# mehta-lab/VisCy

Measured on AMD Instinct MI355X. Metric: training patches/sec (Z=5, 256x256, 1->2ch UNeXt2), higher is better.
Workload: dtype bf16; 1 GPU; UNeXt2 2.5D convnextv2_tiny Z=5 256x256 1->2ch, fwd+MixedLoss(0.5,0,0.5)+bwd+AdamW; per_gpu_batch=512, global_batch=512, parallelism=dp1

## Files before the change

### include/vsx.h

```cpp
#ifndef VSX_H
#define VSX_H
#include <stddef.h>
#include <stdint.h>

#ifdef __cplusplus
extern "C" {
#endif

typedef void* vsx_stream_t;

#define VSX_F32 0
#define VSX_BF16 1

int32_t vsx_version(void);
const char* vsx_last_error(void);
const char* vsx_last_kernel(void);
int32_t vsx_set_flag(const char* name, int32_t value);
int32_t vsx_get_flag(const char* name);
int32_t vsx_det_workspace(float* ws, int64_t floats);
int32_t vsx_det_scope(int32_t on);
int32_t vsx_det_active(void);

#define VSX_A_ROWS 0
#define VSX_A_PATCH2 1
// ... 206 lines not shown
#define VSX_LOSS_SLOT_STRIDE 32
int32_t vsx_loss_tmax(const float* T, int64_t n, float* tmax, vsx_stream_t stream);
int32_t vsx_ssim_scale_fwd_fused(const float* P, const float* T, const float* tmax, float* sum_ssim, float* sum_cs, float* dmu,
                                 float* Po, float* To, float* tmax_next, float* l1sum, float* l2sum, int32_t B, int32_t C,
                                 int32_t D, int32_t H, int32_t W, int32_t last, vsx_stream_t stream);
int32_t vsx_loss_finalize(const float* sum_ssim, const float* sum_cs, const float* l1sum, const float* l2sum,
    const float* npix, float nelem, int32_t B, int32_t nscale, int32_t sum_slots, float a1, float a2, float a3,
    const float* gout, float* loss, float* coef, float* ms_out, vsx_stream_t stream);

int32_t vsx_ln_fwd(const void* x, void* y, float* mean, float* rstd, const float* gamma, const float* beta,
    int32_t rows, int32_t C, float eps, int32_t dtype, vsx_stream_t stream);

int32_t vsx_ln_bwd(const void* dy, const void* x, const float* mean, const float* rstd, const float* gamma,
    const void* add, void* dx, float* dgamma, float* dbeta, int32_t rows, int32_t C, int32_t dtype,
    vsx_stream_t stream);

int32_t vsx_grn_scale(const float* colsq, const float* gamma, float* s, int32_t nb, int32_t N, float eps,
    vsx_stream_t stream);

int32_t vsx_grn_bwd_stats(const float* colsq, const float* P, const float* Sb, const float* gamma, float* t,
    float* dgamma, float* dbeta, float* rowst, int32_t nb, int32_t N, float eps, vsx_stream_t stream);

int32_t vsx_grn_gelu_bwd(void* dz, const void* h, const float* s, const float* t, float* colsum, float* ws,
    int32_t ws_rows, int32_t M, int32_t N, int32_t hw, int32_t dtype, vsx_stream_t stream);

int32_t vsx_adamw(float* p, const float* g, float* m, float* v, const float* hyper, int64_t n,
    vsx_stream_t stream);

int32_t vsx_mlp_supported(int32_t C, int32_t hw, int64_t M, int32_t dtype);
int64_t vsx_mlp_det_floats(int32_t C, int32_t hw, int64_t M, int32_t mode);
// ... 197 lines not shown
```

### viscy_amd/_lib.py

```python

from __future__ import annotations

import ctypes as C
import os

import torch

_HERE = os.path.dirname(os.path.abspath(__file__))
LIB_PATH = os.environ.get("VSX_LIB", os.path.join(_HERE, "libvsx.so"))

VSX_F32, VSX_BF16 = 0, 1
A_ROWS, A_PATCH2, A_CONV3 = 0, 1, 2
PRO_NONE, PRO_GRN = 0, 1
EPI_NONE, EPI_BIAS, EPI_BIAS_GELU_SQ, EPI_BIAS_RES, EPI_DZ, EPI_BIAS_STATS, EPI_LN_BWD = 0, 1, 2, 3, 4, 5, 6
LOSS_SLOTS, LOSS_SLOT_STRIDE = 64, 32
SPOTLIGHT_CHUNK = 16384
SPOTLIGHT_THRESHOLD, SPOTLIGHT_MASK_U8, SPOTLIGHT_MASK_F32 = 0, 1, 2
SPOTLIGHT_WS_FWD, SPOTLIGHT_WS_OTSU = 0, 1

_I32, _F32, _P, _I64 = C.c_int32, C.c_float, C.c_void_p, C.c_int64


class VsxGemm(C.Structure):
    _fields_ = [
# ... 35 lines not shown
    "vsx_version": (_I32, []),
    "vsx_weight_tasks": (_I32, [_P, _I32, _P]),
    "vsx_last_error": (C.c_char_p, []),
    "vsx_last_kernel": (C.c_char_p, []),
    "vsx_set_flag": (_I32, [C.c_char_p, _I32]),
    "vsx_get_flag": (_I32, [C.c_char_p]),
    "vsx_det_workspace": (_I32, [_P, _I64]),
    "vsx_det_scope": (_I32, [_I32]),
    "vsx_det_active": (_I32, []),
    "vsx_gemm_nt": (_I32, [C.POINTER(VsxGemm), _I32, _P]),
    "vsx_gemm_tn": (_I32, [C.POINTER(VsxGemm), _I32, _P]),
    "vsx_gemm_plan": (_I32, [_I32, C.POINTER(VsxGemm), _I32, C.POINTER(VsxGemmPlan)]),
    "vsx_gemm_nt_ln_bwd_supported": (_I32, [_I64, _I32, _I32, _I32]),
    "vsx_ln_fwd": (_I32, [_P, _P, _P, _P, _P, _P, _I32, _I32, _F32, _I32, _P]),
    "vsx_ln_bwd": (_I32, [_P, _P, _P, _P, _P, _P, _P, _P, _P, _I32, _I32, _I32, _P]),
    "vsx_grn_scale": (_I32, [_P, _P, _P, _I32, _I32, _F32, _P]),
    "vsx_grn_bwd_stats": (_I32, [_P, _P, _P, _P, _P, _P, _P, _P, _I32, _I32, _F32, _P]),
    "vsx_grn_gelu_bwd": (_I32, [_P, _P, _P, _P, _P, _P, _I32, _I32, _I32, _I32, _I32, _P]),
    "vsx_dwconv7_fwd": (_I32, [_P, _P, _P, _P, _P, _I32, _I32, _I32, _I32, _I32, _P]),
    "vsx_dwconv7_bwd_data": (_I32, [_P, _P, _P, _P, _I32, _I32, _I32, _I32, _I32, _P]),
    "vsx_dwconv7_bwd_weight": (_I32, [_P, _P, _P, _P, _P, _I32, _I32, _I32, _I32, _I32, _I32, _P]),
    "vsx_stem_im2col": (_I32, [_P, _P, _P, _P, _I32, _I32, _I32, _I32, _I32, _I32, _I32, _I32, _I32, _P]),
    "vsx_stem_im2col_ld": (_I32, [_P, _P, _P, _P, _I32, _I32, _I32, _I32, _I32, _I32, _I32, _I32, _I32, _I32, _P]),
    "vsx_pad_cols": (_I32, [_P, _P, _I32, _I32, _I32, _I32, _P]),
    "vsx_im2col3x3": (_I32, [_P, _P, _I32, _I32, _I32, _I32, _I32, _P]),
    "vsx_col2im3x3": (_I32, [_P, _P, _I32, _I32, _I32, _I32, _I32, _P]),
    "vsx_pixel_shuffle_cat_fwd": (_I32, [_P, _P, _P, _I32, _I32, _I32, _I32, _I32, _I32, _P]),
    "vsx_pixel_shuffle_cat_bwd": (_I32, [_P, _P, _P, _I32, _I32, _I32, _I32, _I32, _I32, _P]),
    "vsx_head_shuffle_fwd": (_I32, [_P, _P, _I32, _I32, _I32, _I32, _I32, _I32, _I32, _P]),
    "vsx_head_shuffle_bwd": (_I32, [_P, _P, _I32, _I32, _I32, _I32, _I32, _I32, _I32, _P]),
# ... 179 lines not shown
```

### viscy_amd/csrc/dwconv.hip

```cpp
#include "vsx_common.h"
#include "../../include/vsx.h"

template <typename T, int NCV, int TH, int TW, int K, bool FLIP>
__global__ __launch_bounds__(256) void dwconv7_kernel(const T* __restrict__ x, const float* __restrict__ w,
                                                      const float* __restrict__ bias, const T* __restrict__ add,
                                                      T* __restrict__ y, int B, int H, int W, int C) {
  constexpr int VN = VT<T>::N;
  constexpr int CB = NCV * VN;
  constexpr int PITCH = CB * (int)sizeof(T) + 16;
  constexpr int IH = TH + 6, IW = TW + 6;
  constexpr int SPR = TW / K;
  static_assert(NCV * TH * SPR == 256, "thread mapping");
  typedef typename VT<T>::vec vec;
  __shared__ __attribute__((aligned(16))) char tile[IH * IW * PITCH];
  __shared__ __attribute__((aligned(16))) float wl[49 * CB];

  const int ncb = (C + CB - 1) / CB;
  const int tiles_x = (W + TW - 1) / TW, tiles_y = (H + TH - 1) / TH;
  int bid = blockIdx.x;
  if ((gridDim.x & 7) == 0) bid = (bid & 7) * (gridDim.x >> 3) + (bid >> 3);
  const int cb = bid % ncb; bid /= ncb;
  const int tx = bid % tiles_x; bid /= tiles_x;
  const int ty = bid % tiles_y;
  const int b = bid / tiles_y;
// ... 59 lines not shown
      const int gx = x0 + sx * K + o;
      if (gx < W) {
        const size_t off = (((size_t)b * H + gy) * W + gx) * C + c0;
        if (add) {
          float a[VN];
          unpack<T>(ldvec<T>(add + off), a);
#pragma unroll
          for (int j = 0; j < VN; ++j) acc[o][j] += a[j];
        }
        stvec<T>(y + off, pack<T>(acc[o]));
      }
    }
  }
}


template <typename T, int NCV, int TH, int TW>
__global__ __launch_bounds__(256) void dwconv7_wgrad_kernel(const T* __restrict__ dy, const T* __restrict__ x,
                                                            float* __restrict__ ws, int B, int H, int W, int C,
                                                            int ngroups) {
  constexpr int VN = VT<T>::N;
  constexpr int CB = NCV * VN;
  constexpr int PITCH = CB * (int)sizeof(T) + 16;
  constexpr int IH = TH + 6, IW = TW + 6;
  constexpr int XT_BYTES = IH * IW * PITCH, DT_BYTES = TH * TW * PITCH;
  static_assert(NCV * 7 * TH <= 256, "thread mapping");
  typedef typename VT<T>::vec vec;
  constexpr int CR = 2;
  constexpr int PART_BYTES = CR * 50 * CB * 4;
  constexpr int SMEM_BYTES = XT_BYTES + DT_BYTES > PART_BYTES ? XT_BYTES + DT_BYTES : PART_BYTES;
  __shared__ __attribute__((aligned(16))) char smem[SMEM_BYTES];
  char* xt = smem;
// ... 7 lines not shown
  const int tiles_x = (W + TW - 1) / TW, tiles_y = (H + TH - 1) / TH;
  const int ntiles = B * tiles_y * tiles_x;

  const int cv = threadIdx.x % NCV;
  const int ky = (threadIdx.x / NCV) % 7;
  const int row = threadIdx.x / (NCV * 7);
  const bool worker = row < TH;
  float acc[7][VN], bsum[VN];
#pragma unroll
  for (int k = 0; k < 7; ++k)
#pragma unroll
    for (int j = 0; j < VN; ++j) acc[k][j] = 0.f;
#pragma unroll
  for (int j = 0; j < VN; ++j) bsum[j] = 0.f;

  for (int tile = group; tile < ntiles; tile += ngroups) {
    int t = tile;
    const int tx = t % tiles_x; t /= tiles_x;
    const int ty = t % tiles_y;
    const int b = t / tiles_y;
    const int y0 = ty * TH, x0 = tx * TW;
    __syncthreads();
    for (int i = threadIdx.x; i < IH * IW * NCV; i += 256) {
      const int c = i % NCV, p = i / NCV;
      const int ix = p % IW, iy = p / IW;
      const int gy = y0 + iy - 3, gx = x0 + ix - 3;
      vec v = vzero<T>();
      if (gy >= 0 && gy < H && gx >= 0 && gx < W && c_base + c * VN < C)
        v = ldvec<T>(x + (((size_t)b * H + gy) * W + gx) * C + c_base + c * VN);
      *reinterpret_cast<vec*>(xt + p * PITCH + c * 16) = v;
    }
    for (int i = threadIdx.x; i < TH * TW * NCV; i += 256) {
      const int c = i % NCV, p = i / NCV;
      const int ix = p % TW, iy = p / TW;
      const int gy = y0 + iy, gx = x0 + ix;
      vec v = vzero<T>();
      if (gy < H && gx < W && c_base + c * VN < C)
        v = ldvec<T>(dy + (((size_t)b * H + gy) * W + gx) * C + c_base + c * VN);
      *reinterpret_cast<vec*>(dt + p * PITCH + c * 16) = v;
    }
    __syncthreads();
    if (worker) {
      const char* xr = xt + ((row + ky) * IW) * PITCH + cv * 16;
      const char* dr = dt + (row * TW) * PITCH + cv * 16;
      float win[7][VN];
#pragma unroll
      for (int i = 0; i < 6; ++i) unpack<T>(*reinterpret_cast<const vec*>(xr + i * PITCH), win[i]);
#pragma unroll 1
      for (int ob = 0; ob < TW; ob += 7) {
#pragma unroll
        for (int u = 0; u < 7; ++u) {
          const int o = ob + u;
          if (o < TW) {
            unpack<T>(*reinterpret_cast<const vec*>(xr + (o + 6) * PITCH), win[(u + 6) % 7]);
            float d[VN];
            unpack<T>(*reinterpret_cast<const vec*>(dr + o * PITCH), d);
            if (ky == 3) {
#pragma unroll
              for (int j = 0; j < VN; ++j) bsum[j] += d[j];
            }
#pragma unroll
            for (int kx = 0; kx < 7; ++kx)
#pragma unroll
              for (int j = 0; j < VN; ++j) acc[kx][j] = fmaf(d[j], win[(u + kx) % 7][j], acc[kx][j]);
          }
        }
      }
    }
  }
  float* part = reinterpret_cast<float*>(smem);
  constexpr int NV = (50 * CB + 255) / 256;
  float tot[NV];
#pragma unroll
  for (int q = 0; q < NV; ++q) tot[q] = 0.f;
  for (int r0 = 0; r0 < TH; r0 += CR) {
    __syncthreads();
    if (worker && row >= r0 && row < r0 + CR) {
      float* pr = part + (size_t)(row - r0) * 50 * CB;
#pragma unroll
      for (int kx = 0; kx < 7; ++kx)
#pragma unroll
        for (int j = 0; j < VN; j += 4)
          *reinterpret_cast<float4*>(pr + (ky * 7 + kx) * CB + cv * VN + j) =
// ... 51 lines not shown
}

template <typename T, int NCV, int TH, int TW, int K>
static int dw_launch_cfg(const void* x, const float* w, const float* bias, const void* add, void* y, int B, int H, int W,
                         int C, bool flip, hipStream_t s) {
  constexpr int CB = NCV * VT<T>::N;
  long blocks = (long)B * vsx_cdiv(H, TH) * vsx_cdiv(W, TW) * vsx_cdiv(C, CB);
  dim3 grid((unsigned)blocks);
  if (flip)
    hipLaunchKernelGGL((dwconv7_kernel<T, NCV, TH, TW, K, true>), grid, dim3(256), 0, s, (const T*)x, w, bias,
                       (const T*)add, (T*)y, B, H, W, C);
  else
    hipLaunchKernelGGL((dwconv7_kernel<T, NCV, TH, TW, K, false>), grid, dim3(256), 0, s, (const T*)x, w, bias,
                       (const T*)add, (T*)y, B, H, W, C);
  VSX_LAUNCH_CHECK();
  return 0;
}

template <typename T>
static int dw_launch(const void* x, const float* w, const float* bias, const void* add, void* y, int B, int H, int W,
                     int C, bool flip, hipStream_t s);
int vsx_dwconv7_mfma_try(const void* x, const float* w, const float* bias, const void* add, void* y, int B, int H, int W, int C,
                         bool flip, hipStream_t s, int* taken);
int vsx_dwconv7_wgrad_mfma_try(const void* dy, const void* x, float* ws, int ws_rows, int B, int H, int W, int C,
                               hipStream_t s, int* taken);
template <>
int dw_launch<bf16_t>(const void* x, const float* w, const float* bias, const void* add, void* y, int B, int H, int W,
                      int C, bool flip, hipStream_t s) {
  int taken = 0;
  if (int rc = vsx_dwconv7_mfma_try(x, w, bias, add, y, B, H, W, C, flip, s, &taken)) return rc;
  if (taken) return 0;
  if (W >= 24) return dw_launch_cfg<bf16_t, 4, 8, 32, 4>(x, w, bias, add, y, B, H, W, C, flip, s);
  return dw_launch_cfg<bf16_t, 8, 8, 8, 2>(x, w, bias, add, y, B, H, W, C, flip, s);
}
template <>
int dw_launch<float>(const void* x, const float* w, const float* bias, const void* add, void* y, int B, int H, int W,
                     int C, bool flip, hipStream_t s) {
  if (W >= 24) return dw_launch_cfg<float, 8, 4, 32, 4>(x, w, bias, add, y, B, H, W, C, flip, s);
  return dw_launch_cfg<float, 8, 8, 8, 2>(x, w, bias, add, y, B, H, W, C, flip, s);
}

extern "C" int32_t vsx_dwconv7_fwd(const void* x, const float* w, const float* bias, const void* add, void* y, int32_t B,
                                   int32_t H, int32_t W, int32_t C, int32_t dtype, vsx_stream_t stream) {
  int vn = dtype == VSX_BF16 ? 8 : 4;
  VSX_CHECK(x && w && y && B > 0 && H > 0 && W > 0 && C > 0 && C % vn == 0, "vsx_dwconv7_fwd: bad arguments (C=%d)", C);
  return dtype == VSX_BF16 ? dw_launch<bf16_t>(x, w, bias, add, y, B, H, W, C, false, (hipStream_t)stream)
                           : dw_launch<float>(x, w, bias, add, y, B, H, W, C, false, (hipStream_t)stream);
}
extern "C" int32_t vsx_dwconv7_bwd_data(const void* dy, const float* w, const void* add, void* dx, int32_t B, int32_t H,
                                        int32_t W, int32_t C, int32_t dtype, vsx_stream_t stream) {
  int vn = dtype == VSX_BF16 ? 8 : 4;
  VSX_CHECK(dy && w && dx && B > 0 && H > 0 && W > 0 && C > 0 && C % vn == 0, "vsx_dwconv7_bwd_data: bad arguments");
  return dtype == VSX_BF16 ? dw_launch<bf16_t>(dy, w, nullptr, add, dx, B, H, W, C, true, (hipStream_t)stream)
                           : dw_launch<float>(dy, w, nullptr, add, dx, B, H, W, C, true, (hipStream_t)stream);
}
template <typename T, int NCV, int TH, int TW>
static int dw_wgrad_cfg(const void* dy, const void* x, float* dw, float* db, float* ws, int ws_rows, int B, int H, int W,
                        int C, hipStream_t st) {
  constexpr int CB = NCV * VT<T>::N;
  const int ncb = vsx_cdiv(C, CB);
  const int ntiles = B * vsx_cdiv(H, TH) * vsx_cdiv(W, TW);
  int ngroups = ntiles < ws_rows ? ntiles : ws_rows;
  if ((long)ngroups * ncb > 4096) ngroups = (int)(4096 / ncb) > 0 ? (int)(4096 / ncb) : 1;
  hipLaunchKernelGGL((dwconv7_wgrad_kernel<T, NCV, TH, TW>), dim3(ngroups * ncb), dim3(256), 0, st, (const T*)dy,
                     (const T*)x, ws, B, H, W, C, ngroups);
  VSX_LAUNCH_CHECK();
  hipLaunchKernelGGL(dw_reduce_rows_kernel, dim3(vsx_cdiv(50 * C, 64), vsx_cdiv(ngroups, 64)), dim3(256), 0, st, ws, dw, db,
                     ngroups, C);
  VSX_LAUNCH_CHECK();
  return 0;
}

extern "C" int32_t vsx_dwconv7_bwd_weight(const void* dy, const void* x, float* dw, float* db, float* ws, int32_t ws_rows,
                                          int32_t B, int32_t H, int32_t W, int32_t C, int32_t dtype,
                                          vsx_stream_t stream) {
  int vn = dtype == VSX_BF16 ? 8 : 4;
  VSX_CHECK(dy && x && dw && ws && ws_rows > 0 && B > 0 && H > 0 && W > 0 && C > 0 && C % vn == 0,
            "vsx_dwconv7_bwd_weight: bad arguments");
  hipStream_t st = (hipStream_t)stream;
  if (dtype == VSX_BF16) {
    int rows = 0;
    if (int rc = vsx_dwconv7_wgrad_mfma_try(dy, x, ws, ws_rows, B, H, W, C, st, &rows)) return rc;
    if (rows > 0) {
      hipLaunchKernelGGL(dw_reduce_rows_kernel, dim3(vsx_cdiv(50 * C, 64), vsx_cdiv(rows, 64)), dim3(256), 0, st, ws, dw, db, rows,
                         C);
      VSX_LAUNCH_CHECK();
      return 0;
    }
    if (W >= 24) return dw_wgrad_cfg<bf16_t, 4, 8, 16>(dy, x, dw, db, ws, ws_rows, B, H, W, C, st);
    return dw_wgrad_cfg<bf16_t, 4, 8, 8>(dy, x, dw, db, ws, ws_rows, B, H, W, C, st);
  }
  if (W >= 24) return dw_wgrad_cfg<float, 4, 8, 32>(dy, x, dw, db, ws, ws_rows, B, H, W, C, st);
  return dw_wgrad_cfg<float, 4, 8, 8>(dy, x, dw, db, ws, ws_rows, B, H, W, C, st);
}
```

### viscy_amd/csrc/norm.hip

```cpp
#include "vsx_common.h"
#include "wtasks.h"
#include "../../include/vsx.h"

template <typename T, int G, int CPL>
__global__ __launch_bounds__(256) void ln_fwd_kernel(const T* __restrict__ x, T* __restrict__ y,
                                                     float* __restrict__ mean_out, float* __restrict__ rstd_out,
                                                     const float* __restrict__ gamma, const float* __restrict__ beta,
                                                     int rows, int C, float eps, int iters, int nt) {
  constexpr int VN = VT<T>::N;
  constexpr int R = CPL == 1 ? 4 : (CPL == 2 ? 2 : 1);
  constexpr int RPI = 256 / G;
  const int nch = C / VN;
  const int gl = threadIdx.x % G;
  float gam[CPL][VN], bet[CPL][VN];
#pragma unroll
  for (int i = 0; i < CPL; ++i) {
    const int c = gl + i * G;
#pragma unroll
    for (int j = 0; j < VN; ++j) {
      gam[i][j] = (gamma && c < nch) ? gamma[c * VN + j] : 1.f;
      bet[i][j] = (gamma && c < nch) ? beta[c * VN + j] : 0.f;
    }
  }
  for (int it = 0; it < iters; ++it) {
// ... 53 lines not shown
      if (gl == 0) {
        if (mean_out) mean_out[row] = mean;
        rstd_out[row] = rstd;
      }
#endif
    }
  }
  }
}

template <typename T, int G, int CPL, bool AFF>
__global__ __launch_bounds__(256) void ln_bwd_kernel(const T* __restrict__ dy, const T* __restrict__ x,
                                                     const float* __restrict__ mean, const float* __restrict__ rstd,
                                                     const float* __restrict__ gamma, const T* __restrict__ add,
                                                     T* __restrict__ dx, float* __restrict__ dgamma,
                                                     float* __restrict__ dbeta, int rows, int C, int iters, int nt) {
  constexpr int VN = VT<T>::N;
  const bool g_nt = nt != 0;
  extern __shared__ float red[];
  const int nch = C / VN;
  const int gl = threadIdx.x % G;
  const int rslot = threadIdx.x / G;
  constexpr int RPI = 256 / G;
  if (AFF && dgamma) {
    for (int i = threadIdx.x; i < 2 * C; i += 256) red[i] = 0.f;
    __syncthreads();
  }
  constexpr int CA = AFF ? CPL : 1, VA = AFF ? VN : 1;
  float dg[CA][VA], db[CA][VA], gam[CA][VA];
  if constexpr (AFF) {
#pragma unroll
    for (int i = 0; i < CPL; ++i) {
      int c = gl + i * G;
#pragma unroll
      for (int j = 0; j < VN; ++j) {
        dg[i][j] = 0.f;
        db[i][j] = 0.f;
        gam[i][j] = (gamma && c < nch) ? gamma[c * VN + j] : 1.f;
      }
    }
  }
  typedef typename VT<T>::vec vec;
// ... 59 lines not shown
            float o[VN];
#pragma unroll
            for (int j = 0; j < VN; ++j) o[j] = rs * (g[i][j] - s1 - xh[i][j] * s2);
            if (add) {
              float a[VN];
              unpack<T>(ar[r][i], a);
#pragma unroll
              for (int j = 0; j < VN; ++j) o[j] += a[j];
            }
            stvec<T>(dx + (size_t)row * C + c * VN, pack<T>(o));
          }
        }
      }
    }
  }
  if constexpr (AFF) if (dgamma) {
#pragma unroll
    for (int i = 0; i < CPL; ++i) {
      int c = gl + i * G;
      if (c < nch) {
#pragma unroll
        for (int j = 0; j < VN; ++j) {
          atomicAdd(&red[c * VN + j], dg[i][j]);
          atomicAdd(&red[C + c * VN + j], db[i][j]);
        }
      }
    }
    __syncthreads();
    for (int i = threadIdx.x; i < C; i += 256) {
      atomicAdd(dgamma + i, red[i]);
      atomicAdd(dbeta + i, red[C + i]);
    }
  }
}

template <typename T, int G, int CPL>
static int ln_launch(bool fwd, const void* a0, const void* a1, void* out, float* mean, float* rstd,
                     const float* gamma, const float* beta, const void* add, float* dgamma, float* dbeta, int rows,
                     int C, float eps, hipStream_t s) {
  constexpr int RPI = 256 / G;
  if (fwd) {
    constexpr int R = CPL == 1 ? 4 : (CPL == 2 ? 2 : 1);
    const int fcap = gamma ? (g_vsx_ln_fblk >= 8 ? g_vsx_ln_fblk / 8 : 1) : g_vsx_ln_fblk;
    int iters = vsx_cdiv(rows, RPI * R * fcap);
    if (iters < 1) iters = 1;
    hipLaunchKernelGGL((ln_fwd_kernel<T, G, CPL>), dim3(vsx_cdiv(rows, RPI * R * iters)), dim3(256), 0, s, (const T*)a0,
                       (T*)out, mean, rstd, gamma, beta, rows, C, eps, iters, g_vsx_ln_stream & 2);
  } else {
    int iters = vsx_cdiv(rows, RPI * (dgamma ? g_vsx_ln_ablk : g_vsx_ln_bblk));
    if (iters < 1) iters = 1;
    int grid = vsx_cdiv(rows, RPI * iters);
    size_t sh = dgamma ? 2 * (size_t)C * sizeof(float) : 0;
    if (gamma || dgamma)
      hipLaunchKernelGGL((ln_bwd_kernel<T, G, CPL, true>), dim3(grid), dim3(256), sh, s, (const T*)a0, (const T*)a1,
                         (const float*)mean, (const float*)rstd, gamma, (const T*)add, (T*)out, dgamma, dbeta, rows, C,
                         iters, g_vsx_ln_stream & 1);
    else
      hipLaunchKernelGGL((ln_bwd_kernel<T, G, CPL, false>), dim3(grid), dim3(256), sh, s, (const T*)a0, (const T*)a1,
                         (const float*)mean, (const float*)rstd, gamma, (const T*)add, (T*)out, dgamma, dbeta, rows, C,
                         iters, g_vsx_ln_stream & 1);
  }
  VSX_LAUNCH_CHECK();
  return 0;
}

template <typename T>
static int ln_dispatch(bool fwd, const void* a0, const void* a1, void* out, float* mean, float* rstd,
                       const float* gamma, const float* beta, const void* add, float* dgamma, float* dbeta, int rows,
                       int C, float eps, hipStream_t s) {
  const int nch = C / VT<T>::N;
#define LN_CASE(G, CPL) return ln_launch<T, G, CPL>(fwd, a0, a1, out, mean, rstd, gamma, beta, add, dgamma, dbeta, rows, C, eps, s)
  if (g_vsx_ln_pack && !fwd) {
    if (nch == 24) LN_CASE(8, 3);
    if (nch == 48) LN_CASE(16, 3);
  }
  if (nch <= 4) LN_CASE(4, 1);
  if (nch <= 8) LN_CASE(8, 1);
  if (nch <= 16) LN_CASE(16, 1);
  if (nch <= 32) LN_CASE(32, 1);
  if (nch <= 64) LN_CASE(64, 1);
  if (nch <= 128) LN_CASE(64, 2);
  if (nch <= 192) LN_CASE(64, 3);
  if (nch <= 256) LN_CASE(64, 4);
#undef LN_CASE
  vsx_set_error("layernorm: C=%d too wide (max %d)", C, 256 * VT<T>::N);
  return 1;
// ... 11 lines not shown
             : ln_dispatch<float>(true, x, nullptr, y, mean, rstd, gamma, beta, nullptr, nullptr, nullptr, rows, C, eps, s);
}

extern "C" int32_t vsx_ln_bwd(const void* dy, const void* x, const float* mean, const float* rstd, const float* gamma,
                              const void* add, void* dx, float* dgamma, float* dbeta, int32_t rows, int32_t C,
                              int32_t dtype, vsx_stream_t stream) {
  int vn = dtype == VSX_BF16 ? 8 : 4;
  VSX_CHECK(rows > 0 && C > 0 && C % vn == 0, "vsx_ln_bwd: rows=%d C=%d (C must be a multiple of %d)", rows, C, vn);
  VSX_CHECK(dy && x && rstd && dx, "vsx_ln_bwd: null pointer");
  VSX_CHECK((dgamma == nullptr) == (dbeta == nullptr), "vsx_ln_bwd: dgamma and dbeta must both be set or both NULL");
  hipStream_t s = (hipStream_t)stream;
  return dtype == VSX_BF16 ? ln_dispatch<bf16_t>(false, dy, x, dx, (float*)mean, (float*)rstd, gamma, nullptr, add,
                                                 dgamma, dbeta, rows, C, 0.f, s)
                           : ln_dispatch<float>(false, dy, x, dx, (float*)mean, (float*)rstd, gamma, nullptr, add,
                                                dgamma, dbeta, rows, C, 0.f, s);
}

__global__ __launch_bounds__(256) void grn_scale_kernel(const float* __restrict__ colsq, const float* __restrict__ gamma,
                                                        float* __restrict__ s, int N, float eps) {
  __shared__ float part[4];
  const int b = blockIdx.x;
  float acc = 0.f;
  for (int n = threadIdx.x; n < N; n += 256) acc += sqrtf(colsq[(size_t)b * N + n]);
  acc = wave_sum(acc);
  if ((threadIdx.x & 63) == 0) part[threadIdx.x >> 6] = acc;
  __syncthreads();
  const float m = (part[0] + part[1] + part[2] + part[3]) / (float)N;
  for (int n = threadIdx.x; n < N; n += 256)
    s[(size_t)b * N + n] = 1.f + gamma[n] * sqrtf(colsq[(size_t)b * N + n]) / (m + eps);
}
// ... 13 lines not shown
  a1 = wave_sum(a1);
  if ((threadIdx.x & 63) == 0) { part[0][threadIdx.x >> 6] = a0; part[1][threadIdx.x >> 6] = a1; }
  __syncthreads();
  const float m = (part[0][0] + part[0][1] + part[0][2] + part[0][3]) / (float)N;
  const float sdg = part[1][0] + part[1][1] + part[1][2] + part[1][3];
  const float inv = 1.f / (m + eps);
  for (int n = threadIdx.x; n < N; n += 256) {
    float g = sqrtf(colsq[(size_t)b * N + n]);
    float pn = P[(size_t)b * N + n];
    float dn = gamma[n] * pn;
    float dgv = dn * inv - sdg * inv * inv / (float)N;
    t[(size_t)b * N + n] = g > 0.f ? dgv / g : 0.f;
    wsg[(size_t)b * N + n] = pn * g * inv;
  }
}
__global__ void reduce_rows_kernel(const float* __restrict__ ws, float* __restrict__ out, int R, int N);

__global__ __launch_bounds__(256) void det_group_sum_kernel(const float* __restrict__ ws, int ld, int col0, float* __restrict__ out,
                                                            int groups, int rpg, int N) {
  __shared__ float part[4][64];
  const int g = blockIdx.y, cl = threadIdx.x & 63, slot = threadIdx.x >> 6;
  const int n = blockIdx.x * 64 + cl;
  float acc = 0.f;
  if (n < N) {
    const float* p = ws + (size_t)g * rpg * ld + col0 + n;
    for (int r = slot; r < rpg; r += 4) acc += p[(size_t)r * ld];
  }
  part[slot][cl] = acc;
  __syncthreads();
  if (slot == 0 && n < N) out[(size_t)g * N + n] += (part[0][cl] + part[1][cl]) + (part[2][cl] + part[3][cl]);
}
int vsx_det_group_sum(const float* ws, int ld, int col0, float* out, int groups, int rows_per_group, int N, hipStream_t s) {
// ... 253 lines not shown
```

### viscy_amd/ops.py

```python

from __future__ import annotations

import contextlib
import ctypes as C
import os
import threading
from typing import Sequence

import torch
from torch import Tensor

from . import _lib as L
from ._lib import VsxGemm, VsxGemmPlan, check, dtype_code, lib, ptr, stream


class Scratch:

    def __init__(self, alloc=None):
        self._alloc = alloc or (lambda floats, dev: torch.empty(floats, dtype=torch.float32, device=dev))
        self._tls = threading.local()
        self.held: list = []

    def take(self, dev, floats: int):
        arenas = getattr(self._tls, "arenas", None)
# ... 143 lines not shown


def ln_fwd(x: Tensor, gamma: Tensor | None, beta: Tensor | None, rows: int, Cc: int, eps: float = 1e-6,
           need_mean: bool = True):
    y = torch.empty_like(x)
    mean = torch.empty(rows, dtype=torch.float32, device=x.device) if need_mean else None
    rstd = torch.empty(rows, dtype=torch.float32, device=x.device)
    check(lib().vsx_ln_fwd(ptr(x), ptr(y), ptr(mean), ptr(rstd), ptr(gamma), ptr(beta), rows, Cc, eps,
                           dtype_code(x.dtype), stream()), "ln_fwd")
    return y, mean, rstd


def ln_bwd(dy: Tensor, x: Tensor, mean: Tensor | None, rstd: Tensor, gamma: Tensor | None, add: Tensor | None,
           dgamma: Tensor | None, dbeta: Tensor | None, rows: int, Cc: int) -> Tensor:
    dx = torch.empty_like(dy)
    check(lib().vsx_ln_bwd(ptr(dy), ptr(x), ptr(mean), ptr(rstd), ptr(gamma), ptr(add), ptr(dx), ptr(dgamma),
                           ptr(dbeta), rows, Cc, dtype_code(dy.dtype), stream()), "ln_bwd")
    return dx


def grn_scale(colsq: Tensor, gamma: Tensor, eps: float = 1e-6) -> Tensor:
    s = torch.empty_like(colsq)
    check(lib().vsx_grn_scale(ptr(colsq), ptr(gamma), ptr(s), colsq.shape[0], colsq.shape[1], eps, stream()), "grn_scale")
    return s


def grn_bwd_stats(colsq: Tensor, P: Tensor, gamma: Tensor, dgamma: Tensor, eps: float = 1e-6, Sb: Tensor | None = None,
                  dbeta: Tensor | None = None) -> Tensor:
    t = torch.empty_like(colsq)
    rowst = torch.empty_like(colsq)
    if _BATCH is not None:
        nb, N = colsq.shape
# ... 1004 lines not shown
```

Baseline: 5656 patches/s.

## Add whole-image dwconv kernels for tiny maps and deterministic LN backward workspace

Adds a depthwise 7x7 forward kernel for feature maps of at most 8x8 that keeps one block per channel group and loops over a batch slice. It double-buffers whole images in shared memory and prefetches the next sample's loads during compute. The wgrad kernel gains a similar whole-map mode with register prefetch. LayerNorm backward replaces shared-memory and global atomics for dgamma/dbeta with wave shuffles plus per-block workspace rows and a separate row reduction, which can also be deferred into the batched weight-task queue. The trade is extra launches and workspace traffic in exchange for fewer atomics and better overlap on low-resolution stages.

Measured after the change: 5690 patches/s, median of 6. No clear change (+0.6%).

```diff
diff --git a/include/vsx.h b/include/vsx.h
--- a/include/vsx.h
+++ b/include/vsx.h
@@ -244,6 +244,10 @@
 int32_t vsx_ln_bwd(const void* dy, const void* x, const float* mean, const float* rstd, const float* gamma,
     const void* add, void* dx, float* dgamma, float* dbeta, int32_t rows, int32_t C, int32_t dtype,
     vsx_stream_t stream);
+int32_t vsx_ln_bwd_ws(const void* dy, const void* x, const float* mean, const float* rstd, const float* gamma,
+    const void* add, void* dx, float* dgamma, float* dbeta, float* ws, int64_t ws_floats, int32_t rows, int32_t C,
+    int32_t dtype, vsx_stream_t stream);
+int64_t vsx_ln_bwd_ws_floats(int32_t rows, int32_t C, int32_t dtype);
 
 int32_t vsx_grn_scale(const float* colsq, const float* gamma, float* s, int32_t nb, int32_t N, float eps,
     vsx_stream_t stream);
diff --git a/viscy_amd/_lib.py b/viscy_amd/_lib.py
--- a/viscy_amd/_lib.py
+++ b/viscy_amd/_lib.py
@@ -73,6 +73,8 @@
     "vsx_gemm_nt_ln_bwd_supported": (_I32, [_I64, _I32, _I32, _I32]),
     "vsx_ln_fwd": (_I32, [_P, _P, _P, _P, _P, _P, _I32, _I32, _F32, _I32, _P]),
     "vsx_ln_bwd": (_I32, [_P, _P, _P, _P, _P, _P, _P, _P, _P, _I32, _I32, _I32, _P]),
+    "vsx_ln_bwd_ws": (_I32, [_P] * 10 + [_I64, _I32, _I32, _I32, _P]),
+    "vsx_ln_bwd_ws_floats": (_I64, [_I32, _I32, _I32]),
     "vsx_grn_scale": (_I32, [_P, _P, _P, _I32, _I32, _F32, _P]),
     "vsx_grn_bwd_stats": (_I32, [_P, _P, _P, _P, _P, _P, _P, _P, _I32, _I32, _F32, _P]),
     "vsx_grn_gelu_bwd": (_I32, [_P, _P, _P, _P, _P, _P, _I32, _I32, _I32, _I32, _I32, _P]),
diff --git a/viscy_amd/csrc/dwconv.hip b/viscy_amd/csrc/dwconv.hip
--- a/viscy_amd/csrc/dwconv.hip
+++ b/viscy_amd/csrc/dwconv.hip
@@ -97,8 +97,139 @@
   }
 }
 
-
-template <typename T, int NCV, int TH, int TW>
+template <typename T, int NCV, int TH, int TW, int K, bool FLIP>
+__global__ __launch_bounds__(256) void dwconv7_map_kernel(const T* __restrict__ x, const float* __restrict__ w,
+                                                          const float* __restrict__ bias, const T* __restrict__ add,
+                                                          T* __restrict__ y, int B, int H, int W, int C, int nsplit) {
+  constexpr int VN = VT<T>::N;
+  constexpr int CB = NCV * VN;
+  constexpr int PITCH = CB * (int)sizeof(T) + 16;
+  constexpr int IH = TH + 6, IW = TW + 6;
+  constexpr int SPR = TW / K;
+  constexpr int TILE_BYTES = IH * IW * PITCH;
+  constexpr int NQ = (TH * TW * NCV + 255) / 256;
+  static_assert(NCV * TH * SPR == 256, "thread mapping");
+  typedef typename VT<T>::vec vec;
+  __shared__ __attribute__((aligned(16))) char tile[2 * TILE_BYTES];
+  __shared__ __attribute__((aligned(16))) float wl[49 * CB];
+
+  const int ncb = (C + CB - 1) / CB;
+  const int cb = blockIdx.x % ncb, part = blockIdx.x / ncb;
+  const int c_base = cb * CB;
+  const int b_lo = (int)((long)B * part / nsplit), b_hi = (int)((long)B * (part + 1) / nsplit);
+
+  for (int i = threadIdx.x; i < 49 * CB; i += 256) {
+    const int t = i / CB, c = i - t * CB;
+    const int tap = FLIP ? 48 - t : t;
+    wl[i] = (c_base + c < C) ? w[(size_t)tap * C + c_base + c] : 0.f;
+  }
+  for (int i = threadIdx.x; i < 2 * IH * IW * NCV; i += 256)
+    *reinterpret_cast<vec*>(tile + (i / NCV) * PITCH + (i % NCV) * 16) = vzero<T>();
+
+  int goff[NQ], loff[NQ];
+#pragma unroll
+  for (int q = 0; q < NQ; ++q) {
+    const int i = threadIdx.x + q * 256;
+    const int c = i % NCV, p = i / NCV;
+    const int ix = p % W, iy = p / W;
+    const bool ok = p < H * W && c_base + c * VN < C;
+    goff[q] = ok ? p * C + c_base + c * VN : -1;
+    loff[q] = ((iy + 3) * IW + ix + 3) * PITCH + c * 16;
+  }
+  const int cv = threadIdx.x % NCV;
+  const int pt = threadIdx.x / NCV;
+  const int sx = pt % SPR, sy = pt / SPR;
+  const int c0 = c_base + cv * VN;
+  const bool orow = sy < H && c0 < C;
+  float bia[VN];
+#pragma unroll
+  for (int j = 0; j < VN; ++j) bia[j] = (bias && c0 + j < C) ? bias[c0 + j] : 0.f;
+
+  const size_t sample = (size_t)H * W * C;
+  vec xq[NQ], aq[K];
+  auto request = [&](int b, vec (&xv)[NQ], vec (&av)[K]) {
+    const T* xs = x + (size_t)b * sample;
+#pragma unroll
+    for (int q = 0; q < NQ; ++q)
+      if (goff[q] >= 0) xv[q] = ldvec<T>(xs + goff[q]);
+    if (add && orow) {
+#pragma unroll
+      for (int o = 0; o < K; ++o)
+        if (sx * K + o < W) av[o] = ldvec<T>(add + (size_t)b * sample + (size_t)(sy * W + sx * K + o) * C + c0);
+    }
+  };
+  if (b_lo < b_hi) request(b_lo, xq, aq);
+  __syncthreads();
+  if (b_lo < b_hi) {
+#pragma unroll
+    for (int q = 0; q < NQ; ++q)
+      if (goff[q] >= 0) *reinterpret_cast<vec*>(tile + loff[q]) = xq[q];
+  }
+  __syncthreads();
+
+  for (int b = b_lo; b < b_hi; ++b) {
+    const char* cur = tile + ((b - b_lo) & 1) * TILE_BYTES;
+    char* nxt = tile + (((b - b_lo) & 1) ^ 1) * TILE_BYTES;
+    vec xn[NQ], an[K];
+    if (b + 1 < b_hi) request(b + 1, xn, an);
+
+    float acc[K][VN];
+#pragma unroll
+    for (int o = 0; o < K; ++o)
+#pragma unroll
+      for (int j = 0; j < VN; ++j) acc[o][j] = bia[j];
+#pragma unroll 1
+    for (int ky = 0; ky < 7; ++ky) {
+      float wk[7][VN];
+#pragma unroll
+      for (int kx = 0; kx < 7; ++kx)
+#pragma unroll
+        for (int j = 0; j < VN; j += 4) {
+          float4 t = *reinterpret_cast<const float4*>(wl + (ky * 7 + kx) * CB + cv * VN + j);
+          wk[kx][j] = t.x; wk[kx][j + 1] = t.y; wk[kx][j + 2] = t.z; wk[kx][j + 3] = t.w;
+        }
+      const char* rowp = cur + ((sy + ky) * IW + sx * K) * PITCH + cv * 16;
+#pragma unroll
+      for (int i = 0; i < K + 6; ++i) {
+        float v[VN];
+        unpack<T>(*reinterpret_cast<const vec*>(rowp + i * PITCH), v);
+#pragma unroll
+        for (int kx = 0; kx < 7; ++kx) {
+          const int o = i - kx;
+          if (o >= 0 && o < K) {
+#pragma unroll
+            for (int j = 0; j < VN; ++j) acc[o][j] = fmaf(v[j], wk[kx][j], acc[o][j]);
+          }
+        }
+      }
+    }
+    if (orow) {
+#pragma unroll
+      for (int o = 0; o < K; ++o) {
+        const int gx = sx * K + o;
+        if (gx < W) {
+          if (add) {
+            float a[VN];
+            unpack<T>(aq[o], a);
+#pragma unroll
+            for (int j = 0; j < VN; ++j) acc[o][j] += a[j];
+          }
+          stvec<T>(y + (size_t)b * sample + (size_t)(sy * W + gx) * C + c0, pack<T>(acc[o]));
+        }
+      }
+    }
+    if (b + 1 < b_hi) {
+#pragma unroll
+      for (int q = 0; q < NQ; ++q)
+        if (goff[q] >= 0) *reinterpret_cast<vec*>(nxt + loff[q]) = xn[q];
+#pragma unroll
+      for (int o = 0; o < K; ++o) aq[o] = an[o];
+    }
+    __syncthreads();
+  }
+}
+
+template <typename T, int NCV, int TH, int TW, bool MAP>
 __global__ __launch_bounds__(256) void dwconv7_wgrad_kernel(const T* __restrict__ dy, const T* __restrict__ x,
                                                             float* __restrict__ ws, int B, int H, int W, int C,
                                                             int ngroups) {
@@ -136,12 +267,50 @@
 #pragma unroll
   for (int j = 0; j < VN; ++j) bsum[j] = 0.f;
 
+  constexpr int NQ = MAP ? (TH * TW * NCV + 255) / 256 : 1;
+  int goff[NQ], xoff[NQ], doff[NQ];
+  vec xq[NQ], dq[NQ];
+  auto request = [&](int b) {
+    const size_t so = (size_t)b * H * W * C;
+#pragma unroll
+    for (int q = 0; q < NQ; ++q)
+      if (goff[q] >= 0) {
+        xq[q] = ldvec<T>(x + so + goff[q]);
+        dq[q] = ldvec<T>(dy + so + goff[q]);
+      }
+  };
+  if constexpr (MAP) {
+    for (int i = threadIdx.x; i < (IH * IW + TH * TW) * NCV; i += 256)
+      *reinterpret_cast<vec*>(smem + (i / NCV) * PITCH + (i % NCV) * 16) = vzero<T>();
+#pragma unroll
+    for (int q = 0; q < NQ; ++q) {
+      const int i = threadIdx.x + q * 256;
+      const int c = i % NCV, p = i / NCV;
+      const int ix = p % W, iy = p / W;
+      goff[q] = (p < H * W && c_base + c * VN < C) ? p * C + c_base + c * VN : -1;
+      xoff[q] = ((iy + 3) * IW + ix + 3) * PITCH + c * 16;
+      doff[q] = (iy * TW + ix) * PITCH + c * 16;
+    }
+    if (group < ntiles) request(group);
+    __syncthreads();
+  }
   for (int tile = group; tile < ntiles; tile += ngroups) {
+    if constexpr (MAP) {
+#pragma unroll
+      for (int q = 0; q < NQ; ++q)
+        if (goff[q] >= 0) {
+          *reinterpret_cast<vec*>(xt + xoff[q]) = xq[q];
+          *reinterpret_cast<vec*>(dt + doff[q]) = dq[q];
+        }
+      __syncthreads();
+      if (tile + ngroups < ntiles) request(tile + ngroups);
+    }
     int t = tile;
     const int tx = t % tiles_x; t /= tiles_x;
     const int ty = t % tiles_y;
     const int b = t / tiles_y;
     const int y0 = ty * TH, x0 = tx * TW;
+    if constexpr (!MAP) {
     __syncthreads();
     for (int i = threadIdx.x; i < IH * IW * NCV; i += 256) {
       const int c = i % NCV, p = i / NCV;
@@ -162,6 +331,7 @@
       *reinterpret_cast<vec*>(dt + p * PITCH + c * 16) = v;
     }
     __syncthreads();
+    }
     if (worker) {
       const char* xr = xt + ((row + ky) * IW) * PITCH + cv * 16;
       const char* dr = dt + (row * TW) * PITCH + cv * 16;
@@ -189,6 +359,7 @@
         }
       }
     }
+    if constexpr (MAP) __syncthreads();
   }
   float* part = reinterpret_cast<float*>(smem);
   constexpr int NV = (50 * CB + 255) / 256;
@@ -270,6 +441,27 @@
     hipLaunchKernelGGL((dwconv7_kernel<T, NCV, TH, TW, K, false>), grid, dim3(256), 0, s, (const T*)x, w, bias,
                        (const T*)add, (T*)y, B, H, W, C);
   VSX_LAUNCH_CHECK();
+  g_vsx_last_kernel = "dwconv7_tile";
+  return 0;
+}
+
+template <typename T, int NCV, int TH, int TW, int K>
+static int dw_launch_map(const void* x, const float* w, const float* bias, const void* add, void* y, int B, int H, int W,
+                         int C, bool flip, hipStream_t s) {
+  constexpr int CB = NCV * VT<T>::N;
+  const int ncb = vsx_cdiv(C, CB);
+  int nsplit = 512 / ncb;
+  if (nsplit > B) nsplit = B;
+  if (nsplit < 1) nsplit = 1;
+  dim3 grid((unsigned)(ncb * nsplit));
+  if (flip)
+    hipLaunchKernelGGL((dwconv7_map_kernel<T, NCV, TH, TW, K, true>), grid, dim3(256), 0, s, (const T*)x, w, bias,
+                       (const T*)add, (T*)y, B, H, W, C, nsplit);
+  else
+    hipLaunchKernelGGL((dwconv7_map_kernel<T, NCV, TH, TW, K, false>), grid, dim3(256), 0, s, (const T*)x, w, bias,
+                       (const T*)add, (T*)y, B, H, W, C, nsplit);
+  VSX_LAUNCH_CHECK();
+  g_vsx_last_kernel = "dwconv7_map";
   return 0;
 }
 
@@ -285,7 +477,11 @@
                       int C, bool flip, hipStream_t s) {
   int taken = 0;
   if (int rc = vsx_dwconv7_mfma_try(x, w, bias, add, y, B, H, W, C, flip, s, &taken)) return rc;
-  if (taken) return 0;
+  if (taken) {
+    g_vsx_last_kernel = "dwconv7_mfma";
+    return 0;
+  }
+  if (H <= 8 && W <= 8) return dw_launch_map<bf16_t, 8, 8, 8, 2>(x, w, bias, add, y, B, H, W, C, flip, s);
   if (W >= 24) return dw_launch_cfg<bf16_t, 4, 8, 32, 4>(x, w, bias, add, y, B, H, W, C, flip, s);
   return dw_launch_cfg<bf16_t, 8, 8, 8, 2>(x, w, bias, add, y, B, H, W, C, flip, s);
 }
@@ -293,6 +489,7 @@
 int dw_launch<float>(const void* x, const float* w, const float* bias, const void* add, void* y, int B, int H, int W,
                      int C, bool flip, hipStream_t s) {
   if (W >= 24) return dw_launch_cfg<float, 8, 4, 32, 4>(x, w, bias, add, y, B, H, W, C, flip, s);
+  if (H <= 8 && W <= 8) return dw_launch_map<float, 8, 8, 8, 2>(x, w, bias, add, y, B, H, W, C, flip, s);
   return dw_launch_cfg<float, 8, 8, 8, 2>(x, w, bias, add, y, B, H, W, C, flip, s);
 }
 
@@ -318,9 +515,15 @@
   const int ntiles = B * vsx_cdiv(H, TH) * vsx_cdiv(W, TW);
   int ngroups = ntiles < ws_rows ? ntiles : ws_rows;
   if ((long)ngroups * ncb > 4096) ngroups = (int)(4096 / ncb) > 0 ? (int)(4096 / ncb) : 1;
-  hipLaunchKernelGGL((dwconv7_wgrad_kernel<T, NCV, TH, TW>), dim3(ngroups * ncb), dim3(256), 0, st, (const T*)dy,
-                     (const T*)x, ws, B, H, W, C, ngroups);
+  const bool map = H <= TH && W <= TW;
+  if (map)
+    hipLaunchKernelGGL((dwconv7_wgrad_kernel<T, NCV, TH, TW, true>), dim3(ngroups * ncb), dim3(256), 0, st, (const T*)dy,
+                       (const T*)x, ws, B, H, W, C, ngroups);
+  else
+    hipLaunchKernelGGL((dwconv7_wgrad_kernel<T, NCV, TH, TW, false>), dim3(ngroups * ncb), dim3(256), 0, st, (const T*)dy,
+                       (const T*)x, ws, B, H, W, C, ngroups);
   VSX_LAUNCH_CHECK();
+  g_vsx_last_kernel = map ? "dwconv7_wgrad_map" : "dwconv7_wgrad_tile";
   hipLaunchKernelGGL(dw_reduce_rows_kernel, dim3(vsx_cdiv(50 * C, 64), vsx_cdiv(ngroups, 64)), dim3(256), 0, st, ws, dw, db,
                      ngroups, C);
   VSX_LAUNCH_CHECK();
@@ -341,6 +544,7 @@
       hipLaunchKernelGGL(dw_reduce_rows_kernel, dim3(vsx_cdiv(50 * C, 64), vsx_cdiv(rows, 64)), dim3(256), 0, st, ws, dw, db, rows,
                          C);
       VSX_LAUNCH_CHECK();
+      g_vsx_last_kernel = "dwconv7_wgrad_mfma";
       return 0;
     }
     if (W >= 24) return dw_wgrad_cfg<bf16_t, 4, 8, 16>(dy, x, dw, db, ws, ws_rows, B, H, W, C, st);
diff --git a/viscy_amd/csrc/norm.hip b/viscy_amd/csrc/norm.hip
--- a/viscy_amd/csrc/norm.hip
+++ b/viscy_amd/csrc/norm.hip
@@ -91,7 +91,8 @@
                                                      const float* __restrict__ mean, const float* __restrict__ rstd,
                                                      const float* __restrict__ gamma, const T* __restrict__ add,
                                                      T* __restrict__ dx, float* __restrict__ dgamma,
-                                                     float* __restrict__ dbeta, int rows, int C, int iters, int nt) {
+                                                     float* __restrict__ dbeta, float* __restrict__ ws, int rows, int C,
+                                                     int iters, int nt) {
   constexpr int VN = VT<T>::N;
   const bool g_nt = nt != 0;
   extern __shared__ float red[];
@@ -99,10 +100,6 @@
   const int gl = threadIdx.x % G;
   const int rslot = threadIdx.x / G;
   constexpr int RPI = 256 / G;
-  if (AFF && dgamma) {
-    for (int i = threadIdx.x; i < 2 * C; i += 256) red[i] = 0.f;
-    __syncthreads();
-  }
   constexpr int CA = AFF ? CPL : 1, VA = AFF ? VN : 1;
   float dg[CA][VA], db[CA][VA], gam[CA][VA];
   if constexpr (AFF) {
@@ -192,30 +189,59 @@
       }
     }
   }
-  if constexpr (AFF) if (dgamma) {
-#pragma unroll
-    for (int i = 0; i < CPL; ++i) {
-      int c = gl + i * G;
-      if (c < nch) {
-#pragma unroll
-        for (int j = 0; j < VN; ++j) {
-          atomicAdd(&red[c * VN + j], dg[i][j]);
-          atomicAdd(&red[C + c * VN + j], db[i][j]);
+  if constexpr (AFF) if (dgamma || ws) {
+#pragma unroll
+    for (int i = 0; i < CPL; ++i)
+#pragma unroll
+      for (int j = 0; j < VN; ++j)
+#pragma unroll
+        for (int o = G; o < 64; o <<= 1) {
+          dg[i][j] += __shfl_xor(dg[i][j], o, 64);
+          db[i][j] += __shfl_xor(db[i][j], o, 64);
+        }
+    if ((threadIdx.x & 63) < G) {
+      float* part = red + (threadIdx.x >> 6) * 2 * C;
+#pragma unroll
+      for (int i = 0; i < CPL; ++i) {
+        const int c = gl + i * G;
+        if (c < nch) {
+#pragma unroll
+          for (int j = 0; j < VN; ++j) {
+            part[c * VN + j] = dg[i][j];
+            part[C + c * VN + j] = db[i][j];
+          }
         }
       }
     }
     __syncthreads();
-    for (int i = threadIdx.x; i < C; i += 256) {
-      atomicAdd(dgamma + i, red[i]);
-      atomicAdd(dbeta + i, red[C + i]);
-    }
-  }
-}
+    float* wg = ws ? ws + (size_t)blockIdx.x * C : dgamma;
+    float* wb = ws ? ws + ((size_t)gridDim.x + blockIdx.x) * C : dbeta;
+    for (int i = threadIdx.x; i < 2 * C; i += 256) {
+      const float v = (red[i] + red[2 * C + i]) + (red[4 * C + i] + red[6 * C + i]);
+      float* o = i < C ? wg + i : wb + (i - C);
+      if (ws)
+        *o = v;
+      else
+        atomicAdd(o, v);
+    }
+  }
+}
+
+__global__ void reduce_rows_kernel(const float* __restrict__ ws, float* __restrict__ out, int R, int N);
+
+struct LnWs {
+  float* ws;
+  int64_t floats;
+  int64_t* need;
+};
+#ifndef VSX_LN_WS_CAP
+#define VSX_LN_WS_CAP 2048
+#endif
 
 template <typename T, int G, int CPL>
 static int ln_launch(bool fwd, const void* a0, const void* a1, void* out, float* mean, float* rstd,
                      const float* gamma, const float* beta, const void* add, float* dgamma, float* dbeta, int rows,
-                     int C, float eps, hipStream_t s) {
+                     int C, float eps, hipStream_t s, const LnWs* w) {
   constexpr int RPI = 256 / G;
   if (fwd) {
     constexpr int R = CPL == 1 ? 4 : (CPL == 2 ? 2 : 1);
@@ -225,18 +251,31 @@
     hipLaunchKernelGGL((ln_fwd_kernel<T, G, CPL>), dim3(vsx_cdiv(rows, RPI * R * iters)), dim3(256), 0, s, (const T*)a0,
                        (T*)out, mean, rstd, gamma, beta, rows, C, eps, iters, g_vsx_ln_stream & 2);
   } else {
-    int iters = vsx_cdiv(rows, RPI * (dgamma ? g_vsx_ln_ablk : g_vsx_ln_bblk));
+    int iters = vsx_cdiv(rows, RPI * (w ? VSX_LN_WS_CAP : dgamma ? g_vsx_ln_ablk : g_vsx_ln_bblk));
     if (iters < 1) iters = 1;
     int grid = vsx_cdiv(rows, RPI * iters);
-    size_t sh = dgamma ? 2 * (size_t)C * sizeof(float) : 0;
-    if (gamma || dgamma)
+    if (w && w->need) {
+      *w->need = 2 * (int64_t)grid * C;
+      return 0;
+    }
+    VSX_CHECK(!w || (w->ws && w->floats >= 2 * (int64_t)grid * C), "vsx_ln_bwd_ws: workspace needs %ld floats (vsx_ln_bwd_ws_floats)",
+              (long)(2 * (int64_t)grid * C));
+    float* ws = w ? w->ws : nullptr;
+    size_t sh = (dgamma || ws) ? 8 * (size_t)C * sizeof(float) : 0;
+    if (gamma || dgamma || ws)
       hipLaunchKernelGGL((ln_bwd_kernel<T, G, CPL, true>), dim3(grid), dim3(256), sh, s, (const T*)a0, (const T*)a1,
-                         (const float*)mean, (const float*)rstd, gamma, (const T*)add, (T*)out, dgamma, dbeta, rows, C,
+                         (const float*)mean, (const float*)rstd, gamma, (const T*)add, (T*)out, dgamma, dbeta, ws, rows, C,
                          iters, g_vsx_ln_stream & 1);
     else
       hipLaunchKernelGGL((ln_bwd_kernel<T, G, CPL, false>), dim3(grid), dim3(256), sh, s, (const T*)a0, (const T*)a1,
-                         (const float*)mean, (const float*)rstd, gamma, (const T*)add, (T*)out, dgamma, dbeta, rows, C,
+                         (const float*)mean, (const float*)rstd, gamma, (const T*)add, (T*)out, dgamma, dbeta, ws, rows, C,
                          iters, g_vsx_ln_stream & 1);
+    if (ws && dgamma) {
+      VSX_LAUNCH_CHECK();
+      const dim3 rg(vsx_cdiv(C, 64), vsx_cdiv(grid, 64));
+      hipLaunchKernelGGL(reduce_rows_kernel, rg, dim3(256), 0, s, (const float*)ws, dgamma, grid, C);
+      hipLaunchKernelGGL(reduce_rows_kernel, rg, dim3(256), 0, s, (const float*)(ws + (size_t)grid * C), dbeta, grid, C);
+    }
   }
   VSX_LAUNCH_CHECK();
   return 0;
@@ -245,9 +284,9 @@
 template <typename T>
 static int ln_dispatch(bool fwd, const void* a0, const void* a1, void* out, float* mean, float* rstd,
                        const float* gamma, const float* beta, const void* add, float* dgamma, float* dbeta, int rows,
-                       int C, float eps, hipStream_t s) {
+                       int C, float eps, hipStream_t s, const LnWs* w = nullptr) {
   const int nch = C / VT<T>::N;
-#define LN_CASE(G, CPL) return ln_launch<T, G, CPL>(fwd, a0, a1, out, mean, rstd, gamma, beta, add, dgamma, dbeta, rows, C, eps, s)
+#define LN_CASE(G, CPL) return ln_launch<T, G, CPL>(fwd, a0, a1, out, mean, rstd, gamma, beta, add, dgamma, dbeta, rows, C, eps, s, w)
   if (g_vsx_ln_pack && !fwd) {
     if (nch == 24) LN_CASE(8, 3);
     if (nch == 48) LN_CASE(16, 3);
@@ -289,6 +328,33 @@
                                                  dgamma, dbeta, rows, C, 0.f, s)
                            : ln_dispatch<float>(false, dy, x, dx, (float*)mean, (float*)rstd, gamma, nullptr, add,
                                                 dgamma, dbeta, rows, C, 0.f, s);
+}
+
+extern "C" int64_t vsx_ln_bwd_ws_floats(int32_t rows, int32_t C, int32_t dtype) {
+  int vn = dtype == VSX_BF16 ? 8 : 4;
+  if (rows <= 0 || C <= 0 || C % vn) return 0;
+  int64_t need = 0;
+  LnWs w{nullptr, 0, &need};
+  int rc = dtype == VSX_BF16 ? ln_dispatch<bf16_t>(false, nullptr, nullptr, nullptr, nullptr, nullptr, nullptr, nullptr, nullptr,
+                                                   nullptr, nullptr, rows, C, 0.f, nullptr, &w)
+                             : ln_dispatch<float>(false, nullptr, nullptr, nullptr, nullptr, nullptr, nullptr, nullptr, nullptr,
+                                                  nullptr, nullptr, rows, C, 0.f, nullptr, &w);
+  return rc ? 0 : need;
+}
+
+extern "C" int32_t vsx_ln_bwd_ws(const void* dy, const void* x, const float* mean, const float* rstd, const float* gamma,
+                                 const void* add, void* dx, float* dgamma, float* dbeta, float* ws, int64_t ws_floats,
+                                 int32_t rows, int32_t C, int32_t dtype, vsx_stream_t stream) {
+  int vn = dtype == VSX_BF16 ? 8 : 4;
+  VSX_CHECK(rows > 0 && C > 0 && C % vn == 0, "vsx_ln_bwd_ws: rows=%d C=%d (C must be a multiple of %d)", rows, C, vn);
+  VSX_CHECK(dy && x && rstd && dx && ws, "vsx_ln_bwd_ws: null pointer");
+  VSX_CHECK((dgamma == nullptr) == (dbeta == nullptr), "vsx_ln_bwd_ws: dgamma and dbeta must both be set or both NULL");
+  hipStream_t s = (hipStream_t)stream;
+  LnWs w{ws, ws_floats, nullptr};
+  return dtype == VSX_BF16 ? ln_dispatch<bf16_t>(false, dy, x, dx, (float*)mean, (float*)rstd, gamma, nullptr, add, dgamma,
+                                                 dbeta, rows, C, 0.f, s, &w)
+                           : ln_dispatch<float>(false, dy, x, dx, (float*)mean, (float*)rstd, gamma, nullptr, add, dgamma,
+                                                dbeta, rows, C, 0.f, s, &w);
 }
 
 __global__ __launch_bounds__(256) void grn_scale_kernel(const float* __restrict__ colsq, const float* __restrict__ gamma,
@@ -332,8 +398,6 @@
     wsg[(size_t)b * N + n] = pn * g * inv;
   }
 }
-__global__ void reduce_rows_kernel(const float* __restrict__ ws, float* __restrict__ out, int R, int N);
-
 __global__ __launch_bounds__(256) void det_group_sum_kernel(const float* __restrict__ ws, int ld, int col0, float* __restrict__ out,
                                                             int groups, int rpg, int N) {
   __shared__ float part[4][64];
diff --git a/viscy_amd/ops.py b/viscy_amd/ops.py
--- a/viscy_amd/ops.py
+++ b/viscy_amd/ops.py
@@ -181,8 +181,24 @@
 def ln_bwd(dy: Tensor, x: Tensor, mean: Tensor | None, rstd: Tensor, gamma: Tensor | None, add: Tensor | None,
            dgamma: Tensor | None, dbeta: Tensor | None, rows: int, Cc: int) -> Tensor:
     dx = torch.empty_like(dy)
-    check(lib().vsx_ln_bwd(ptr(dy), ptr(x), ptr(mean), ptr(rstd), ptr(gamma), ptr(add), ptr(dx), ptr(dgamma),
-                           ptr(dbeta), rows, Cc, dtype_code(dy.dtype), stream()), "ln_bwd")
+    dc = dtype_code(dy.dtype)
+    if dgamma is None:
+        check(lib().vsx_ln_bwd(ptr(dy), ptr(x), ptr(mean), ptr(rstd), ptr(gamma), ptr(add), ptr(dx), None, None, rows, Cc, dc,
+                               stream()), "ln_bwd")
+        return dx
+    nws = int(lib().vsx_ln_bwd_ws_floats(rows, Cc, dc))
+    if nws <= 0:
+        raise RuntimeError(f"ln_bwd: rows={rows} C={Cc} {dy.dtype} is not served")
+    args = (ptr(dy), ptr(x), ptr(mean), ptr(rstd), ptr(gamma), ptr(add), ptr(dx))
+    if _BATCH is not None:
+        ws = torch.empty(nws, dtype=torch.float32, device=dy.device)
+        check(lib().vsx_ln_bwd_ws(*args, None, None, ptr(ws), nws, rows, Cc, dc, stream()), "ln_bwd_ws")
+        R = nws // (2 * Cc)
+        _queue(L.WTASK_REDUCE_ROWS, 0, (R, Cc), ws[:R * Cc], dgamma, None, None)
+        _queue(L.WTASK_REDUCE_ROWS, 0, (R, Cc), ws[R * Cc:], dbeta, None, None)
+        return dx
+    ws = _workspace(dy.device, nws)
+    check(lib().vsx_ln_bwd_ws(*args, ptr(dgamma), ptr(dbeta), ptr(ws), nws, rows, Cc, dc, stream()), "ln_bwd_ws")
     return dx
 
 
```
